# pavlidic/Binary-SpGEMM

Hardware: AMD Instinct MI355X
Metric: output nnz/sec (GNZ/s) (higher is better)
Workload: dtype int32

## Files before the change

binary-spgemm_amd/bspgemm/__init__.py:

```python
import ctypes as C
import os
import subprocess
import weakref

import numpy as np

os.environ.setdefault("OMP_NUM_THREADS", str(min(16, len(os.sched_getaffinity(0)))))
os.environ.setdefault("GPU_MAX_HW_QUEUES", "8")

_PKG = os.path.dirname(os.path.abspath(__file__))
_ROOT = os.path.dirname(_PKG)
LIB_PATH = os.path.join(_ROOT, "libbspgemm.so")

_I32P = np.ctypeslib.ndpointer(dtype=np.int32, flags="C_CONTIGUOUS")
_I64P = np.ctypeslib.ndpointer(dtype=np.int64, flags="C_CONTIGUOUS")

STATUS = {0: "OK", 1: "ERR_INVALID", 2: "ERR_ALLOC", 3: "ERR_HIP", 4: "ERR_NO_DEVICE",
          5: "ERR_OVERFLOW", 6: "ERR_IO", 7: "ERR_FORMAT", 8: "ERR_COMM", 9: "ERR_SIZE"}

EXPORTS = [
    "bspgemm_status_string", "bspgemm_last_error", "bspgemm_create", "bspgemm_destroy",
    "bspgemm_set_stream", "bspgemm_synchronize", "bspgemm_matrix_upload", "bspgemm_matrix_wrap_device",
    "bspgemm_matrix_free", "bspgemm_matrix_rows", "bspgemm_matrix_cols", "bspgemm_matrix_nnz",
    "bspgemm_multiply", "bspgemm_multiply_masked", "bspgemm_result_rows", "bspgemm_result_nnz",
    "bspgemm_result_row_ptr_device", "bspgemm_result_col_idx_device", "bspgemm_result_download",
    "bspgemm_result_free", "bspgemm_row_work_prefix", "bspgemm_partition_rows", "bspgemm_last_stats",
    "SpGEMM_hip", "SpGEMM_hip_bigslice", "SpGEMM_hip_mat", "SpGEMM_hip_masked", "bspgemm_dropin_set_device",
    "bspgemm_comm_unique_id", "bspgemm_comm_create", "bspgemm_comm_destroy", "bspgemm_comm_stitch_row_ptr", "bspgemm_lengths_to_row_ptr",
    "bspgemm_readCOO", "bspgemm_write_mtx", "bspgemm_write_result_mtx", "bspgemm_csr_equal",
    "bspgemm_csr_equal64", "bspgemm_gen_uniform", "bspgemm_gen_rmat", "bspgemm_gen_powerlaw",
    "bspgemm_matrix_from_result", "bspgemm_closure",
    "bspgemm_readCOO_ex", "bspgemm_comm_create_host", "bspgemm_comm_rank", "bspgemm_comm_size",
    "bspgemm_comm_gather_col_idx", "SpGEMM_hip_multi", "bspgemm_device_count", "bspgemm_stats_at",
    "bspgemm_set_flow", "bspgemm_set_class_timing", "bspgemm_build_info", "bspgemm_matrix_invalidate", "bspgemm_comm_agree", "bspgemm_comm_inject_failure",
    "bspgemm_set_option", "bspgemm_get_option", "bspgemm_matrix_uses_blocked_table", "bspgemm_matrix_uses_padded_rows",
]


class BspgemmError(RuntimeError):
    def __init__(self, status, where=""):
        self.status = status
        msg = lib().bspgemm_last_error().decode(errors="replace") if _lib is not None else ""
        super().__init__("%s: %s %s" % (where, STATUS.get(status, status), msg))


MAX_BINS = 20
FLOWS = {"auto": 0, "upper-bound": 1, "exact": 2}
OPTIONS = {"class_streams": 1, "blocked_extents": 2, "check": 3, "small_path": 4, "padded_rows": 5}


class Stats(C.Structure):
    _fields_ = [("rows", C.c_int64), ("nnz_a", C.c_int64), ("products", C.c_int64), ("nnz_c", C.c_int64),
                ("bytes_alg", C.c_int64), ("bytes_read_alg", C.c_int64), ("rows_per_bin", C.c_int64 * MAX_BINS),
                ("ms_total", C.c_float), ("ms_symbolic", C.c_float), ("ms_prepass", C.c_float),
                ("ms_count", C.c_float), ("ms_numeric", C.c_float), ("ms_stitch", C.c_float),
                ("ms_bin", C.c_float * MAX_BINS), ("ms_bin_count", C.c_float * MAX_BINS),
                ("t_bin", C.c_float * MAX_BINS), ("t_bin_count", C.c_float * MAX_BINS), ("bins", C.c_int),
                ("bin_cap", C.c_int * MAX_BINS), ("flow", C.c_int), ("prepass_kernel", C.c_int),
                ("class_streams", C.c_int), ("small_path", C.c_int), ("checked", C.c_int), ("padded_rows", C.c_int)]
# ... 60 lines not shown
    L.bspgemm_set_stream.argtypes = [VP, VP]
    L.bspgemm_synchronize.argtypes = [VP]
    L.bspgemm_set_flow.argtypes = [VP, C.c_int]
    L.bspgemm_set_class_timing.argtypes = [VP, C.c_int]
    L.bspgemm_build_info.restype = C.c_char_p
    L.bspgemm_matrix_invalidate.argtypes = [VP]
    L.bspgemm_set_option.argtypes = [VP, C.c_int, C.c_int]
    L.bspgemm_get_option.argtypes = [VP, C.c_int]
    L.bspgemm_matrix_uses_blocked_table.argtypes = [VP]
    L.bspgemm_matrix_uses_padded_rows.argtypes = [VP]
    L.bspgemm_matrix_upload.argtypes = [VP, C.c_int, C.c_int, VP, VP, PVP]
    L.bspgemm_matrix_wrap_device.argtypes = [VP, C.c_int, C.c_int, C.c_int64, VP, VP, PVP]
    L.bspgemm_matrix_free.argtypes = [VP]
    L.bspgemm_matrix_free.restype = None
    L.bspgemm_matrix_rows.argtypes = [VP]
    L.bspgemm_matrix_cols.argtypes = [VP]
    L.bspgemm_matrix_nnz.argtypes = [VP]
    L.bspgemm_matrix_nnz.restype = C.c_int64
    L.bspgemm_multiply.argtypes = [VP, VP, VP, C.c_int, C.c_int, PVP]
    L.bspgemm_multiply_masked.argtypes = [VP, VP, VP, VP, C.c_int, C.c_int, PVP]
    L.bspgemm_result_rows.argtypes = [VP]
    L.bspgemm_result_nnz.argtypes = [VP]
    L.bspgemm_result_nnz.restype = C.c_int64
    L.bspgemm_result_row_ptr_device.argtypes = [VP]
    L.bspgemm_result_row_ptr_device.restype = VP
    L.bspgemm_result_col_idx_device.argtypes = [VP]
    L.bspgemm_result_col_idx_device.restype = VP
    L.bspgemm_result_download.argtypes = [VP, VP, VP, VP]
    L.bspgemm_result_free.argtypes = [VP]
    L.bspgemm_result_free.restype = None
    L.bspgemm_matrix_from_result.argtypes = [VP, VP, C.c_int, PVP]
    L.bspgemm_closure.argtypes = [VP, VP, C.c_int, PVP, C.POINTER(C.c_int)]
    L.bspgemm_row_work_prefix.argtypes = [VP, VP, VP, _I64P]
    L.bspgemm_partition_rows.argtypes = [VP, VP, VP, C.c_int, _I32P]
    L.bspgemm_last_stats.argtypes = [VP, C.POINTER(Stats)]
    L.bspgemm_stats_at.argtypes = [VP, C.c_int, C.POINTER(Stats)]
    IPP = C.POINTER(C.POINTER(C.c_int))
    L.SpGEMM_hip.argtypes = [_I32P, VP, C.c_int, _I32P, _I32P, C.c_int, IPP, _I32P, C.c_int]
    L.SpGEMM_hip_bigslice.argtypes = [_I32P, _I32P, C.c_int, _I32P, _I32P, C.c_int, IPP, _I32P,
                                      C.POINTER(C.c_int), C.c_int, C.c_int]
    L.SpGEMM_hip_mat.argtypes = [_I32P, _I32P, C.c_int, _I32P, _I32P, C.c_int, _I32P, _I32P]
    L.SpGEMM_hip_masked.argtypes = [_I32P, _I32P, C.c_int, _I32P, _I32P, C.c_int, _I32P, _I32P, IPP, _I32P,
                                    C.POINTER(C.c_int)]
    L.bspgemm_dropin_set_device.argtypes = [C.c_int]
    L.bspgemm_comm_unique_id.argtypes = [C.c_char_p]
    L.bspgemm_comm_create.argtypes = [VP, C.c_char_p, C.c_int, C.c_int, PVP]
    L.bspgemm_comm_destroy.argtypes = [VP]
    L.bspgemm_comm_destroy.restype = None
    L.bspgemm_comm_stitch_row_ptr.argtypes = [VP, VP, _I32P, PVP, VP]
    L.bspgemm_lengths_to_row_ptr.argtypes = [VP, VP, C.c_int, C.c_int, _I32P, VP, VP]
    U32PP = C.POINTER(C.POINTER(C.c_uint32))
    L.bspgemm_readCOO.argtypes = [C.c_char_p, U32PP, U32PP, C.POINTER(C.c_uint32), C.POINTER(C.c_uint32),
                                  C.POINTER(C.c_uint32)]
    L.bspgemm_readCOO_ex.argtypes = [C.c_char_p, C.c_uint, U32PP, U32PP, C.POINTER(C.c_uint32), C.POINTER(C.c_uint32),
                                     C.POINTER(C.c_uint32)]
    L.bspgemm_comm_create_host.argtypes = [VP, C.POINTER(HostTransport), C.c_int, C.c_int, PVP]
    L.bspgemm_comm_rank.argtypes = [VP]
    L.bspgemm_comm_size.argtypes = [VP]
    L.bspgemm_comm_gather_col_idx.argtypes = [VP, VP, _I64P, C.c_int, VP]
    L.SpGEMM_hip_multi.argtypes = [VP, _I32P, _I32P, C.c_int, _I32P, _I32P, C.c_int, IPP, _I32P, C.c_int]
    L.bspgemm_write_mtx.argtypes = [C.c_char_p, C.c_int, C.c_int, _I32P, _I32P]
    L.bspgemm_write_result_mtx.argtypes = [C.c_char_p, C.c_int, C.c_int, _I64P, _I32P]
    L.bspgemm_csr_equal.argtypes = [_I32P, _I32P, _I32P, _I32P, C.c_int]
    L.bspgemm_csr_equal64.argtypes = [_I32P, _I64P, _I32P, _I64P, C.c_int]
    L.bspgemm_gen_uniform.argtypes = [C.c_int, C.c_int, C.c_uint64, IPP, IPP]
    L.bspgemm_gen_rmat.argtypes = [C.c_int, C.c_int, C.c_double, C.c_double, C.c_double, C.c_uint64, IPP, IPP]
# ... 142 lines not shown

    def multiply_masked(self, A, B, F, row_begin=0, row_end=None):
        row_end = A.rows if row_end is None else row_end
        r = C.c_void_p()
        _chk(lib().bspgemm_multiply_masked(self._h, A._h, B._h, F._h, row_begin, row_end, C.byref(r)),
             "bspgemm_multiply_masked")
        return Result(self, r)

    def matrix_from_result(self, result, cols):
        m = C.c_void_p()
        _chk(lib().bspgemm_matrix_from_result(self._h, result._h, cols, C.byref(m)), "matrix_from_result")
        return Matrix(self, m, keep=None)

    def closure(self, A, max_iter=64):
        r, it = C.c_void_p(), C.c_int()
        _chk(lib().bspgemm_closure(self._h, A._h, max_iter, C.byref(r), C.byref(it)), "bspgemm_closure")
        return Result(self, r), it.value

    def lengths_to_row_ptr(self, d_lengths, world, width, bounds, d_row_ptr, hip_stream=None):
        b = np.ascontiguousarray(bounds, dtype=np.int32)
        _chk(lib().bspgemm_lengths_to_row_ptr(self._h, C.c_void_p(int(d_lengths)), int(world), int(width), b,
                                              C.c_void_p(int(d_row_ptr)), C.c_void_p(hip_stream or 0)), "lengths_to_row_ptr")

    def stats(self, age=0):
        s = Stats()
        _chk(lib().bspgemm_stats_at(self._h, age, C.byref(s)), "stats_at")
        return s.as_dict()

    def row_work_prefix(self, A, B):
        out = np.zeros(A.rows + 1, dtype=np.int64)
        _chk(lib().bspgemm_row_work_prefix(self._h, A._h, B._h, out), "row_work_prefix")
        return out

    def partition_rows(self, A, B, parts):
        out = np.zeros(parts + 1, dtype=np.int32)
        _chk(lib().bspgemm_partition_rows(self._h, A._h, B._h, parts, out), "partition_rows")
        return out


class Matrix:
    def __init__(self, ctx, handle, keep):
        self.ctx, self._h, self._keep = ctx, handle, keep
        ctx._children.add(self)
        self.rows = lib().bspgemm_matrix_rows(handle)
        self.cols = lib().bspgemm_matrix_cols(handle)
        self.nnz = lib().bspgemm_matrix_nnz(handle)

    def invalidate(self):
        _chk(lib().bspgemm_matrix_invalidate(self._h), "matrix_invalidate")

    @property
    def uses_blocked_table(self):
        return lib().bspgemm_matrix_uses_blocked_table(self._h)

    @property
    def uses_padded_rows(self):
        return lib().bspgemm_matrix_uses_padded_rows(self._h)

    def free(self):
        if self._h:
            lib().bspgemm_matrix_free(self._h)
            self._h = C.c_void_p()

    def __del__(self):
        try:
            self.free()
# ... 79 lines not shown
```

binary-spgemm_amd/csrc/dense_rows.hip:

```cpp
#include "kernels.hpp"
#include "wave.hpp"
#include <stdlib.h>
#include <type_traits>

namespace bsp {

constexpr int kDenseThreadsBig = 1024;
constexpr int kDenseThreadsMid = 512;
constexpr int kMidMinWaves = 8;
constexpr int kBigMinWaves = 4;
constexpr int kDenseMaxWords = 16384;
constexpr int kMidMaxWords = 4096;
constexpr int kDenseWordBits = 12;
constexpr int kDenseQuadsPerThreadBig = 16;
constexpr int kDenseQuadsPerThreadMid = 8;
constexpr int kDenseInFlightBig = 8;
constexpr int kDenseInFlightMid = 4;

struct __attribute__((packed, aligned(4))) Int4U { int x, y, z, w; };
struct __attribute__((packed, aligned(4))) Int2U { int x, y; };

struct GatherState {
    long long QB = 0;
    bool plan_kept = false;
// ... 6 lines not shown
    static constexpr int kTileQ = kThreads * kQPT;
    static constexpr int kTileWords = kTileQ / 32;
    static_assert(kTileWords % 64 == 0 && kTileWords <= kThreads, "one wave scans the tile's words, blocked");
    int wcnt[kWaves];
    long long wsum[kWaves];
    int2 sd[kThreads];
    u32 tb[kTileWords];
    u32 tw[2][kTileWords];
    int tpre[2][kTileWords];
};

template <int kThreads, int kQPT>
__device__ __forceinline__ void gather_init(GatherLds<kThreads, kQPT> &L)
{
    if ((int)threadIdx.x < GatherLds<kThreads, kQPT>::kTileWords) L.tb[threadIdx.x] = 0u;
}

template <int kThreads, int kQPT, int kInFlight, typename Ins>
__device__ __forceinline__ void gather_sweep(GatherLds<kThreads, kQPT> &L, GatherState &g, const int2 *__restrict__ ab,
                                             const int *__restrict__ Bcol, int nnzB, int a0, int a1, bool first_sweep, Ins ins)
{
    using LT = GatherLds<kThreads, kQPT>;
    constexpr int kWaves = LT::kWaves, kTileQ = LT::kTileQ, kTileWords = LT::kTileWords;
    static_assert(kQPT % kInFlight == 0 && kInFlight % 4 == 0, "whole steps; the last step in quarters");
    const int tid = threadIdx.x, lane = tid & 63, wave = tid >> 6;
    int2 e_next = make_int2(0, 0);
    if (!g.plan_kept && a0 + tid < a1) e_next = ab[a0 + tid];
    for (int ja = a0; ja < a1; ja += kThreads) {
        int2 e = make_int2(0, 0);
        int nq = 0, cidx = 0;
        long long qexcl = 0;
        if (!g.plan_kept) {
            e = e_next;
            e_next = make_int2(0, 0);
            if (ja + kThreads + tid < a1) e_next = ab[ja + kThreads + tid];
            nq = (int)(((u32)e.y + 3u) >> 2);
            const int inc = wave_incl_scan(nq);
            const u64 nonempty = __ballot(nq > 0);
            if (lane == 63) L.wsum[wave] = (long long)inc;
            if (lane == 0) L.wcnt[wave] = __popcll(nonempty);
            __syncthreads();
            qexcl = (long long)(inc - nq);
            g.QB = 0;
            cidx = __popcll(nonempty & mask_lt(lane));
            for (int k = 0; k < kWaves; k++) {
                const long long t = L.wsum[k];
                const int c = L.wcnt[k];
                if (k < wave) { qexcl += t; cidx += c; }
                g.QB += t;
            }
            if (nq > 0) L.sd[cidx] = make_int2((int)((u32)e.x - 4u * (u32)qexcl), e.x + e.y);
            if (g.QB == 0) __syncthreads();
        }
        int carry = -1;
        for (long long T0 = 0; T0 < g.QB; T0 += kTileQ) {
            if (!g.plan_kept) {
                g.buf ^= 1;
                if (nq > 0 && qexcl >= T0 && qexcl < T0 + kTileQ) {
                    const int rel = (int)(qexcl - T0);
                    atomicOr(&L.tb[rel >> 5], 1u << (rel & 31));
                }
                __syncthreads();
                if (wave == 0) {
                    constexpr int WPL = kTileWords / 64;
                    u32 x[WPL];
                    int c[WPL], run = 0;
// ... 677 lines not shown
```

binary-spgemm_amd/csrc/kernels.hpp:

```cpp
#pragma once
#include <hip/hip_runtime.h>
#include <stdint.h>
#include <stdlib.h>

namespace bsp {

constexpr int kWaveBins = 16;
constexpr int kNumBins = kWaveBins + 4;
constexpr int kRankBin = kWaveBins + 1;
constexpr int kMidBin = kWaveBins + 2;
constexpr int kDenseBin = kWaveBins + 3;
constexpr int kRankCap = 6144;
int rank_cap_for_cols(long long cols);
constexpr int kMaxBins = 20;
constexpr int kWaveChunks[kWaveBins + 1] = {0, 1, 2, 3, 4, 5, 6, 7, 8, 10, 12, 14, 16, 20, 24, 28, 32};
constexpr int kMaxWaveCap = 64 * kWaveChunks[kWaveBins];
constexpr int kMidCap = 524288;
inline int mid_cap_for_cols(long long cols)
{
    const long long passes = (cols + (1ll << 18) - 1) >> 18;
    if (passes <= 1) return kMidCap;
    const long long c = kMidCap / passes;
    return c < kMaxWaveCap ? kMaxWaveCap : (int)c;
}
constexpr int kRowsPerWave = 16;

constexpr int kWaveTopWords = 256;

inline int levels_for_cols(int64_t cols)
{
    for (int L = 1; L < 5; L++)
        if (cols <= ((int64_t)kWaveTopWords << (5 * L))) return L;
    return 5;
}

constexpr int kWaveTopWordsWide = 512;
inline int wave_levels_for_cols(int64_t cols)
{
    const int L = levels_for_cols(cols);
    if (L == 4 && cols <= ((int64_t)kWaveTopWordsWide << 15)) return 3;
    return L;
}

struct RowRec {
    int row;
    int a0;
    int alen;
    int f;
};

void launch_row_work(const int *Arow, const int *Acol, const int *Brow, const int *Bblk8, const int *Bpad, const int2 *Bext,
                     int row_begin, int row_end, long long *F, int2 *ab, hipStream_t s);
void launch_blk8(const int *row_ptr, const int *start_ptr, int n, int *blk, unsigned long long *clamped_nnz, hipStream_t s);
void launch_pad_lengths(const int *row_ptr, int n, int *plen, hipStream_t s);
void launch_pad_copy(const int *row_ptr, const int *col_idx, const int *pad_ptr, int n, int *col_pad, int2 *ext, hipStream_t s);

void launch_deg8(const int *row_ptr, int n, unsigned char *deg8, hipStream_t s);
void launch_row_products(const int *Arow, const int *Acol, const int *Brow, const unsigned char *Bdeg8,
                         int row_begin, int row_end, long long *F, hipStream_t s);

struct PrepScalars {
    long long totalF;
    long long heavy_total;
    long long products;
    int a_lo, a_hi;
    int bin_count[kNumBins];
};
void launch_scan_and_bin(const long long *F, int n, int row_begin, const int *Arow, long long *prefix,
                         long long *partials, int *bin_tiles, int *bin_count, RowRec *rec,
                         long long *recpre, int *cnt, int heavy_cols, long long *hpartials, int mid_cap, int rank_cap, int bound_cols,
                         hipStream_t s, PrepScalars *scal = nullptr, const long long *true_F = nullptr);

constexpr int kCompactGran = 4096;
inline size_t compact_chunk_rows(long long max_out) { return (size_t)((max_out + kCompactGran - 1) / kCompactGran) + 2; }
void launch_scan_counts(const int *cnt, int n, long long *prefix, long long *partials,
                        const long long *base, hipStream_t s, int *chunk_row = nullptr);

constexpr unsigned kErrCapacity = 1u;
constexpr unsigned kErrStaleTable = 2u;
void launch_wave_rows(int bin, int levels, const int2 *ab, const int *Bcol, int cols,
                      const RowRec *rec, const long long *recpre, const long long *row_ptr, int nrows,
                      int row_begin, int *tmp, int *cnt, unsigned *err, hipStream_t s, bool count_only = false);
// ... 54 lines not shown
```

binary-spgemm_amd/csrc/multiply.hip:

```cpp
#include "internal.hpp"

using namespace bsp;

static bspgemm_status check_operands(bspgemm_context *ctx, const bspgemm_matrix *A, const bspgemm_matrix *B,
                                     int row_begin, int row_end)
{
    if (!ctx || !A || !B) return FAIL(BSPGEMM_ERR_INVALID, "NULL operand");
    if (A->ctx != ctx || B->ctx != ctx) return FAIL(BSPGEMM_ERR_INVALID, "operand belongs to another context");
    if (row_begin < 0 || row_end < row_begin || row_end > A->rows) return FAIL(BSPGEMM_ERR_INVALID, "row range");
    if (B->rows < A->cols) return FAIL(BSPGEMM_ERR_INVALID, "B has fewer rows than A has columns");
    return BSPGEMM_OK;
}


static void class_order(const int *bin_count, long long total_products, int *order, int *lane)
{
    int light[kWaveBins];
    for (int k = 0; k < kWaveBins; k++) light[k] = k + 1;
    const long long heavy_lower_bound = ((long long)bin_count[kRankBin] + bin_count[kMidBin] + bin_count[kDenseBin]) * kMaxWaveCap;
    if (heavy_lower_bound * 8 < total_products) {
        long long key[kNumBins] = {};
        for (int b = 1; b <= kWaveBins; b++) key[b] = (long long)bin_count[b] * kWaveChunks[b];
        for (int a = 1; a < kWaveBins; a++)
            for (int c = a; c > 0 && key[light[c]] > key[light[c - 1]]; c--) {
// ... 521 lines not shown
        C = next;
        if (C->nnz == prev_nnz) break;
        prev_nnz = C->nnz;
        if (it + 1 == max_iter) break;
        bspgemm_matrix *nm = nullptr;
        st = bspgemm_matrix_from_result(ctx, C, n, &nm);
        if (st) break;
        bspgemm_matrix_free(cur);
        cur = nm;
    }
    bspgemm_matrix_free(cur);
    if (st) { bspgemm_result_free(C); return st; }
    *T = C;
    return BSPGEMM_OK;
}

extern "C" bspgemm_status bspgemm_row_work_prefix(bspgemm_context *ctx, const bspgemm_matrix *A,
                                                  const bspgemm_matrix *B, int64_t *prefix_host)
{
    if (!prefix_host) return FAIL(BSPGEMM_ERR_INVALID, "prefix_host is NULL");
    if (bspgemm_status st = check_operands(ctx, A, B, 0, A ? A->rows : 0)) return st;
    if (bspgemm_status st = use_device(ctx)) return st;
    const int R = A->rows;
    if (bspgemm_status st = ensure_rows(ctx, (size_t)R + 1)) return st;
    if (bspgemm_status st = ensure_deg8(B)) return st;
    launch_row_products(A->d_row_ptr, A->d_col_idx, B->d_row_ptr, B->d_deg8, 0, R, ctx->F, ctx->stream);
    launch_scan_and_bin(ctx->F, R, 0, A->d_row_ptr, ctx->Fprefix, ctx->partials, ctx->bin_tiles, ctx->bin_count,
                        ctx->rec, ctx->recpre, ctx->cnt, 0, nullptr, mid_cap_for_cols(B->cols), rank_cap_for_cols(B->cols), 0, ctx->stream);
    HIPCHK(hipMemcpyAsync(prefix_host, ctx->Fprefix, ((size_t)R + 1) * sizeof(long long), hipMemcpyDeviceToHost, ctx->stream));
    HIPCHK(hipStreamSynchronize(ctx->stream));
    return BSPGEMM_OK;
}

extern "C" bspgemm_status bspgemm_partition_rows(bspgemm_context *ctx, const bspgemm_matrix *A,
                                                 const bspgemm_matrix *B, int parts, int *bounds)
{
    if (!bounds || parts <= 0 || !A) return FAIL(BSPGEMM_ERR_INVALID, "partition_rows");
    const int R = A->rows;
    int64_t *prefix = static_cast<int64_t *>(malloc(((size_t)R + 1) * sizeof(int64_t)));
    if (!prefix) return FAIL(BSPGEMM_ERR_ALLOC, "prefix");
    bspgemm_status st = bspgemm_row_work_prefix(ctx, A, B, prefix);
    if (st == BSPGEMM_OK) {
        const long long per_row = 32;
        const long long total = prefix[R] + per_row * R;
        bounds[0] = 0;
        int r = 0;
        for (int p = 1; p < parts; p++) {
            const long long target = total / parts * p;
            while (r < R && prefix[r] + per_row * r < target) r++;
            bounds[p] = r;
        }
        bounds[parts] = R;
    }
    free(prefix);
    return st;
}
```

binary-spgemm_amd/csrc/prepass.hip:

```cpp
#include "kernels.hpp"
#include "wave.hpp"

namespace bsp {

struct __attribute__((packed, aligned(4))) Int2U { int x, y; };

constexpr int kLongRow = 256;
constexpr int kRowWorkUnroll = 4;
template <typename Sweep>
__device__ __forceinline__ long long rows_of_a_wave(int a0, int a1, int sub, Sweep &&sweep)
{
    const int lane = threadIdx.x & 63;
    long long long_sum = 0;
#pragma unroll
    for (int q = 0; q < 8; q++) {
        const int qa0 = __builtin_amdgcn_readlane(a0, q * 8), qa1 = __builtin_amdgcn_readlane(a1, q * 8);
        if (qa1 - qa0 > kLongRow) {
            long long t = sweep((long long)qa0 + lane, (long long)qa1, 64);
#pragma unroll
            for (int d = 1; d < 64; d <<= 1) t += __shfl_xor(t, d, 64);
            if (lane == q * 8) long_sum = t;
        }
    }
    const bool is_long = a1 - a0 > kLongRow;
    long long sum = is_long ? 0ll : sweep((long long)a0 + sub, (long long)a1, 8);
    sum += __shfl_xor(sum, 1, 64);
    sum += __shfl_xor(sum, 2, 64);
    sum += __shfl_xor(sum, 4, 64);
    return is_long ? long_sum : sum;
}

template <bool PAD>
__global__ __launch_bounds__(256) void k_row_work(const int *__restrict__ Arow,
                                                  const int *__restrict__ Acol,
                                                  const int *__restrict__ Brow,
                                                  const int2 *__restrict__ Bext,
                                                  int row_begin, int nrows,
                                                  long long *__restrict__ F,
                                                  int2 *__restrict__ ab)
{
    const long long gid = (long long)blockIdx.x * blockDim.x + threadIdx.x;
    const int r = (int)(gid >> 3);
    const int sub = (int)(gid & 7);
    int a0 = 0, a1 = 0;
    if (r < nrows) { a0 = Arow[row_begin + r]; a1 = Arow[row_begin + r + 1]; }
    constexpr int U = kRowWorkUnroll;
    auto sweep = [&](long long first, long long end, int stride) {
        long long sum = 0;
        for (long long jj = first; jj < end; jj += (long long)stride * U) {
            int j[U];
#pragma unroll
            for (int u = 0; u < U; u++) j[u] = (jj + stride * u < end) ? Acol[jj + stride * u] : -1;
            Int2U pr[U];
#pragma unroll
            for (int u = 0; u < U; u++) {
                pr[u].x = pr[u].y = 0;
                if (j[u] >= 0) {
                    if (PAD) { const int2 e = Bext[j[u]]; pr[u].x = e.x; pr[u].y = e.x + e.y; }
                    else pr[u] = *reinterpret_cast<const Int2U *>(Brow + j[u]);
                }
            }
#pragma unroll
            for (int u = 0; u < U; u++)
                if (j[u] >= 0) {
                    const int len = pr[u].y - pr[u].x;
                    ab[jj + stride * u] = make_int2(pr[u].x, len);
                    sum += (long long)len;
                }
        }
        return sum;
    };
    const long long sum = rows_of_a_wave(a0, a1, sub, sweep);
    if (r < nrows && sub == 0) F[r] = sum;
}

struct __attribute__((packed, aligned(4))) Blk8 { int base; unsigned lo, hi; };

__global__ __launch_bounds__(256) void k_blk8(const int *__restrict__ row_ptr, const int *__restrict__ start_ptr, int n,
                                              int *__restrict__ blk, unsigned long long *__restrict__ clamped_nnz)
{
    const int b = blockIdx.x * blockDim.x + threadIdx.x;
    if (b * 8 >= n) return;
    const int r0 = b * 8;
    unsigned lo = 0u, hi = 0u;
    long long clamped = 0;
    int prev = row_ptr[r0];
    const int base = start_ptr[r0];
#pragma unroll
    for (int k = 0; k < 8; k++) {
        int d = 0;
        if (r0 + k < n) {
            const int nx = row_ptr[r0 + k + 1];
            d = nx - prev;
            prev = nx;
        }
        const unsigned byte = (unsigned)(d < 255 ? d : 255);
        if (d >= 255) clamped += d;
        if (k < 4) lo |= byte << (8 * k); else hi |= byte << (8 * (k - 4));
    }
    if (clamped > 0) atomicAdd(clamped_nnz, (unsigned long long)clamped);
    blk[3 * b] = base;
    blk[3 * b + 1] = (int)lo;
    blk[3 * b + 2] = (int)hi;
}
void launch_blk8(const int *row_ptr, const int *start_ptr, int n, int *blk, unsigned long long *clamped_nnz, hipStream_t s)
{
    if (n <= 0) return;
    const int nb = (n + 7) / 8;
    hipLaunchKernelGGL(k_blk8, dim3((nb + 255) / 256), dim3(256), 0, s, row_ptr, start_ptr ? start_ptr : row_ptr, n, blk, clamped_nnz);
}

template <bool PAD>
__global__ __launch_bounds__(256) void k_row_work_blk(const int *__restrict__ Arow,
                                                      const int *__restrict__ Acol,
                                                      const int *__restrict__ Brow,
                                                      const int *__restrict__ Bblk,
                                                      const int *__restrict__ Bpad,
                                                      int row_begin, int nrows,
                                                      long long *__restrict__ F,
                                                      int2 *__restrict__ ab)
{
    const long long gid = (long long)blockIdx.x * blockDim.x + threadIdx.x;
    const int r = (int)(gid >> 3);
    const int sub = (int)(gid & 7);
    int a0 = 0, a1 = 0;
    if (r < nrows) { a0 = Arow[row_begin + r]; a1 = Arow[row_begin + r + 1]; }
    constexpr int U = kRowWorkUnroll;
    auto sweep = [&](long long first, long long end, int stride) {
        long long sum = 0;
        for (long long jj = first; jj < end; jj += (long long)stride * U) {
            int j[U];
#pragma unroll
            for (int u = 0; u < U; u++) j[u] = (jj + stride * u < end) ? Acol[jj + stride * u] : -1;
            Blk8 w[U];
#pragma unroll
            for (int u = 0; u < U; u++) {
                w[u].base = 0; w[u].lo = w[u].hi = 0u;
                if (j[u] >= 0) w[u] = *reinterpret_cast<const Blk8 *>(Bblk + 3 * (j[u] >> 3));
            }
            int start[U], len[U];
            bool sat[U];
#pragma unroll
            for (int u = 0; u < U; u++) {
                const int k = j[u] & 7;
                const u64 d = ((u64)w[u].hi << 32) | (u64)w[u].lo;
                const u64 below = d & ((1ull << (8 * k)) - 1ull);
                const u64 upto = (k == 7) ? d : (d & ((1ull << (8 * k + 8)) - 1ull));
                const u64 v = ~upto;
                sat[u] = j[u] >= 0 && ((v - 0x0101010101010101ull) & ~v & 0x8080808080808080ull) != 0ull;
                if (PAD) {
                    const u64 m0f = 0x0f0f0f0f0f0f0f0full, m01 = 0x0101010101010101ull;
                    const u64 units = ((below >> 4) & m0f) + ((((below & m0f) + m0f) >> 4) & m01);
                    start[u] = w[u].base + 16 * ((int)__builtin_amdgcn_sad_u8((unsigned)units, 0u, 0u)
                                                 + (int)__builtin_amdgcn_sad_u8((unsigned)(units >> 32), 0u, 0u));
                } else {
                    start[u] = w[u].base + (int)__builtin_amdgcn_sad_u8((unsigned)below, 0u, 0u)
                               + (int)__builtin_amdgcn_sad_u8((unsigned)(below >> 32), 0u, 0u);
                }
                len[u] = (int)((d >> (8 * k)) & 255ull);
            }
            Int2U pr[U];
            int ps[U];
#pragma unroll
            for (int u = 0; u < U; u++) {
                pr[u].x = pr[u].y = 0;
                ps[u] = 0;
                if (sat[u]) {
                    pr[u] = *reinterpret_cast<const Int2U *>(Brow + j[u]);
                    if (PAD) ps[u] = Bpad[j[u]];
                }
            }
#pragma unroll
            for (int u = 0; u < U; u++)
                if (j[u] >= 0) {
                    if (sat[u]) { start[u] = PAD ? ps[u] : pr[u].x; len[u] = pr[u].y - pr[u].x; }
                    ab[jj + stride * u] = make_int2(start[u], len[u]);
                    sum += (long long)len[u];
                }
        }
        return sum;
    };
    const long long sum = rows_of_a_wave(a0, a1, sub, sweep);
    if (r < nrows && sub == 0) F[r] = sum;
}

void launch_row_work(const int *Arow, const int *Acol, const int *Brow, const int *Bblk8, const int *Bpad, const int2 *Bext,
                     int row_begin, int row_end, long long *F, int2 *ab, hipStream_t s)
{
    const int nrows = row_end - row_begin;
    if (nrows <= 0) return;
    const long long threads = (long long)nrows * 8;
    const int grid = (int)((threads + 255) / 256);
    if (Bblk8 && Bpad)
        hipLaunchKernelGGL(k_row_work_blk<true>, dim3(grid), dim3(256), 0, s, Arow, Acol, Brow, Bblk8, Bpad, row_begin, nrows, F, ab);
    else if (Bblk8)
        hipLaunchKernelGGL(k_row_work_blk<false>, dim3(grid), dim3(256), 0, s, Arow, Acol, Brow, Bblk8, nullptr, row_begin, nrows, F, ab);
    else if (Bext)
        hipLaunchKernelGGL(k_row_work<true>, dim3(grid), dim3(256), 0, s, Arow, Acol, Brow, Bext, row_begin, nrows, F, ab);
    else
        hipLaunchKernelGGL(k_row_work<false>, dim3(grid), dim3(256), 0, s, Arow, Acol, Brow, nullptr, row_begin, nrows, F, ab);
}

__global__ __launch_bounds__(256) void k_pad_lengths(const int *__restrict__ row_ptr, int n, int *__restrict__ plen)
{
    const int i = blockIdx.x * blockDim.x + threadIdx.x;
    if (i < n) plen[i] = ((row_ptr[i + 1] - row_ptr[i]) + 15) & ~15;
}
void launch_pad_lengths(const int *row_ptr, int n, int *plen, hipStream_t s)
{
// ... 14 lines not shown
}
void launch_pad_copy(const int *row_ptr, const int *col_idx, const int *pad_ptr, int n, int *col_pad, int2 *ext, hipStream_t s)
{
    if (n <= 0) return;
    const long long threads = (long long)n * 16;
    hipLaunchKernelGGL(k_pad_copy, dim3((unsigned)((threads + 255) / 256)), dim3(256), 0, s, row_ptr, col_idx, pad_ptr, n, col_pad, ext);
}

__global__ __launch_bounds__(256) void k_deg8(const int *__restrict__ row_ptr, int n, unsigned char *__restrict__ deg8)
{
    const int i = blockIdx.x * blockDim.x + threadIdx.x;
    if (i < n) {
        const int d = row_ptr[i + 1] - row_ptr[i];
        deg8[i] = (unsigned char)(d < 255 ? d : 255);
    }
}
void launch_deg8(const int *row_ptr, int n, unsigned char *deg8, hipStream_t s)
{
    if (n <= 0) return;
    hipLaunchKernelGGL(k_deg8, dim3((n + 255) / 256), dim3(256), 0, s, row_ptr, n, deg8);
}

__global__ __launch_bounds__(256) void k_row_products(const int *__restrict__ Arow, const int *__restrict__ Acol,
                                                      const int *__restrict__ Brow,
                                                      const unsigned char *__restrict__ Bdeg8,
                                                      int row_begin, int nrows, long long *__restrict__ F)
{
    const long long gid = (long long)blockIdx.x * blockDim.x + threadIdx.x;
    const int r = (int)(gid >> 3);
    const int sub = (int)(gid & 7);
    int a0 = 0, a1 = 0;
    if (r < nrows) { a0 = Arow[row_begin + r]; a1 = Arow[row_begin + r + 1]; }
    constexpr int U = 4;
    auto sweep = [&](long long first, long long end, int stride) {
        long long sum = 0;
        for (long long jj = first; jj < end; jj += (long long)stride * U) {
            int j[U];
#pragma unroll
            for (int u = 0; u < U; u++) j[u] = (jj + stride * u < end) ? Acol[jj + stride * u] : -1;
            int d[U];
#pragma unroll
            for (int u = 0; u < U; u++) d[u] = j[u] >= 0 ? (int)Bdeg8[j[u]] : 0;
#pragma unroll
            for (int u = 0; u < U; u++) {
                if (d[u] == 255) d[u] = Brow[j[u] + 1] - Brow[j[u]];
                sum += (long long)d[u];
            }
        }
        return sum;
    };
    const long long sum = rows_of_a_wave(a0, a1, sub, sweep);
    if (r < nrows && sub == 0) F[r] = sum;
}

__global__ __launch_bounds__(256) void k_check_tables(const int *__restrict__ row_ptr, int n,
                                                      const unsigned char *__restrict__ deg8, const int *__restrict__ blk,
                                                      const int *__restrict__ pad_ptr, unsigned *__restrict__ err)
{
    const int i = blockIdx.x * blockDim.x + threadIdx.x;
    if (i >= n) return;
    const int d = row_ptr[i + 1] - row_ptr[i];
    const unsigned want = (unsigned)(d < 255 ? d : 255);
    bool bad = d < 0;
    if (deg8) bad = bad || deg8[i] != want;
    if (blk) {
        const int b = i >> 3, k = i & 7;
        const unsigned w = (unsigned)blk[3 * b + 1 + (k >> 2)];
        bad = bad || ((w >> (8 * (k & 3))) & 255u) != want || (k == 0 && blk[3 * b] != (pad_ptr ? pad_ptr[i] : row_ptr[i]));
    }
    if (pad_ptr) bad = bad || pad_ptr[i + 1] - pad_ptr[i] != ((d + 15) & ~15);
    if (bad) atomicOr(err, kErrStaleTable);
}
// ... 328 lines not shown
```

binary-spgemm_amd/csrc/wave_masked.hip:

```cpp
#include "kernels.hpp"
#include "wave.hpp"

namespace bsp {

constexpr int kMaskWinChunks = 4;
constexpr long long kMaskWaveMaxProducts = 8192;

template <int LEVELS, int CHUNKS>
struct MaskCfg {
    static constexpr int CAP = 64 * CHUNKS;
    static constexpr int TOPW = 256;
    static constexpr int bytes_per_wave = 4 * TOPW + 2 * TOPW + 8 * kMaskWinChunks + 4 * 64
                                          + 4 * CAP * 3
                                          + (LEVELS >= 3 ? 4 * CAP + 2 * CAP : 32)
                                          + 0;
    static constexpr int w4 = (4 * bytes_per_wave > 64 * 1024) ? 0 : (160 * 1024 / (4 * bytes_per_wave)) * 4;
    static constexpr int w2 = (2 * bytes_per_wave > 64 * 1024) ? 0 : (160 * 1024 / (2 * bytes_per_wave)) * 2;
    static constexpr int WAVES = (w4 >= w2 && w4 > 0) ? 4 : (w2 > 0 ? 2 : 1);
};

template <int LEVELS, int CHUNKS>
__global__ __launch_bounds__((64 * MaskCfg<LEVELS, CHUNKS>::WAVES))
void k_wave_masked(const int2 *__restrict__ ab, const int *__restrict__ Bcol, int topw,
                   const int *__restrict__ Frow, const int *__restrict__ Fcol,
// ... 78 lines not shown
            const unsigned short *Ppre = topPre;
#pragma unroll
            for (int lev = LEVELS - 2; lev >= 0; lev--) {
                u32 *S = (lev == 1) ? SB : SA;
                unsigned short *Spre = preB;
#pragma unroll
                for (int c = 0; c < CHUNKS; c++) {
                    const bool ok = c * 64 + lane < mlen;
                    const u32 cc = (u32)mcol[c];
                    const u32 x = P[rank[c]];
                    const int pre = Ppre[rank[c]];
                    const u32 b = (cc >> (5 * (lev + 1))) & 31;
                    const int r2 = pre + __popc(x & ((1u << b) - 1u));
                    if (ok) {
                        atomicOr(&S[r2], 1u << ((cc >> (5 * lev)) & 31));
                        if (lev == 0) L0w[r2] = cc >> 5;
                    }
                    rank[c] = r2;
                }
                wave_lds_fence();
                if (lev > 0) {
                    scan_blocked<CHUNKS>(S, Spre, lane);
                    wave_lds_fence();
                    P = S;
                    Ppre = Spre;
                }
            }
            L0 = SA;
        }

        for (int ab0 = 0; ab0 < alen; ab0 += 64) {
            int2 e = make_int2(0, 0);
            if (ab0 + lane < alen) e = ab[a0 + ab0 + lane];
            const int bs = e.x, len = e.y;
            const int inc = wave_incl_scan(len);
            const int excl = inc - len;
            const int Fb = wave_bcast(inc, 63);
            for (int w0 = 0; w0 < Fb; w0 += 64 * PCH) {
                const bool part = len > 0 && excl < w0 + 64 * PCH && excl + len > w0;
                const u64 bal = __ballot(part);
                if (part) {
                    const int sidx = __popcll(bal & mask_lt(lane));
                    const int pos = (excl > w0 ? excl : w0) - w0;
                    delta[sidx] = bs - excl;
                    atomicOr(&starts[pos >> 6], 1ull << (pos & 63));
                }
                wave_lds_fence();
                u64 sw = 0ull;
                if (lane < PCH) { sw = starts[lane]; starts[lane] = 0ull; }
                const int sinc = wave_incl_scan(__popcll(sw));
                const int sbefore = sinc - __popcll(sw);
                int gaddr[PCH];
#pragma unroll
                for (int c = 0; c < PCH; c++) {
                    const int p = c * 64 + lane;
                    const u64 M = wave_bcast64(sw, c);
                    const int before = wave_bcast(sbefore, c);
                    const bool ok = w0 + p < Fb;
                    int s = before + __popcll(M & mask_le(lane)) - 1;
                    s = ok ? s : 0;
                    gaddr[c] = ok ? delta[s] + w0 + p : 0;
                }
                int pc[PCH];
#pragma unroll
                for (int c = 0; c < PCH; c++) {
                    const bool ok = w0 + c * 64 + lane < Fb;
                    pc[c] = ok ? Bcol[gaddr[c]] : -1;
// ... 134 lines not shown
```

binary-spgemm_amd/csrc/wave_rows.inc:

```
#include "kernels.hpp"
#include "wave.hpp"

namespace bsp {

constexpr int waves_per_cu(int w, int bytes) { return (w * bytes > 64 * 1024) ? 0 : (160 * 1024 / (w * bytes)) * w; }

constexpr int prev_wave_chunks(int chunks)
{
    int prev = 0;
    for (int b = 1; b <= kWaveBins; b++) {
        if (kWaveChunks[b] == chunks) return prev;
        prev = kWaveChunks[b];
    }
    return 0;
}

template <int LEVELS, int CHUNKS, int TWP>
struct WaveCfg {
    static constexpr int CAP = 64 * CHUNKS;
    static constexpr int SW = (CHUNKS <= 2) ? CHUNKS : ((CHUNKS + 3) & ~3);
    static constexpr int SLOTS = 64 * SW;
    static constexpr int TOPW = 64 * TWP;
    static constexpr int bytes_per_wave = 4 * TOPW + 2 * TOPW + 8 * CHUNKS + 4 * SLOTS
                                          + (LEVELS >= 2 ? 4 * SLOTS : 16)
// ... 22 lines not shown
    return make_int2((int)(u32)v, (int)(u32)((u64)v >> 32));
}

constexpr int kMaxAmbiguous = 12;
constexpr int wr_floor_log2(int x) { int k = 0; while ((2 << k) <= x) k++; return k; }

template <int LEVELS, int CHUNKS, int TWP, bool COUNT>
__global__ __launch_bounds__((64 * WaveCfg<LEVELS, CHUNKS, TWP>::WAVES))
void k_wave_rows(const int2 *__restrict__ ab, const int *__restrict__ Bcol,
                 const RowRec *__restrict__ rec, const long long *__restrict__ recpre,
                 const long long *__restrict__ row_ptr,
                 int nrows, int rpw, int row_begin, int *__restrict__ tmp, int *__restrict__ cnt,
                 unsigned *__restrict__ err)
{
    using Cfg = WaveCfg<LEVELS, CHUNKS, TWP>;
    constexpr int TOPW = Cfg::TOPW, WAVES = Cfg::WAVES, SW = Cfg::SW, SLOTS = Cfg::SLOTS, FULL = Cfg::FULL;
    __shared__ __attribute__((aligned(16))) u32 s_top[WAVES][TOPW];
    __shared__ __attribute__((aligned(16))) unsigned short s_topPre[WAVES][TOPW];
    __shared__ __attribute__((aligned(16))) u64 s_starts[WAVES][CHUNKS];
    __shared__ __attribute__((aligned(16))) u32 s_L0w[WAVES][SLOTS];
    __shared__ __attribute__((aligned(16))) u32 s_SA[WAVES][LEVELS >= 2 ? SLOTS : 4];
    __shared__ __attribute__((aligned(16))) u32 s_SB[WAVES][LEVELS >= 3 ? SLOTS : 4];
    __shared__ __attribute__((aligned(16))) unsigned short s_preB[WAVES][LEVELS >= 3 ? SLOTS : 8];
    __shared__ __attribute__((aligned(16))) unsigned short s_preA[WAVES][LEVELS >= 4 ? SLOTS : 8];

    const int lane = lane_id();
    const int plane = (int)(__brev((unsigned)lane) >> 26);
    const int wave_in_wg = threadIdx.x >> 6;
    const long long wave_global = (long long)blockIdx.x * WAVES + wave_in_wg;
    const long long k0 = wave_global * rpw;
    if (k0 >= nrows) return;
    const int nmine = (nrows - k0 < rpw) ? (int)(nrows - k0) : rpw;

    int r_row = 0, r_a0 = 0, r_alen = 0;
    long long r_pre = 0;
    if (lane < nmine) {
        const RowRec q = rec[k0 + lane];
        r_row = q.row;
        r_a0 = q.a0;
        r_alen = q.alen;
        if (!COUNT) r_pre = row_ptr ? row_ptr[q.row - row_begin] : recpre[k0 + lane];
    }

    u32 *top = s_top[wave_in_wg];
    unsigned short *topPre = s_topPre[wave_in_wg];
    u64 *starts = s_starts[wave_in_wg];
    u32 *L0w = s_L0w[wave_in_wg];
    int *delta = reinterpret_cast<int *>(s_L0w[wave_in_wg]);
    u32 *SA = s_SA[wave_in_wg];
    u32 *SB = s_SB[wave_in_wg];
    unsigned short *preA = s_preA[wave_in_wg];
    unsigned short *preB = s_preB[wave_in_wg];

    constexpr int TW = TOPW / 64;
    clear_blocked<TW>(top, lane);
    if (lane < CHUNKS) starts[lane] = 0ull;
    if (LEVELS >= 2) clear_blocked<SW>(SA, lane);
    if (LEVELS >= 3) clear_blocked<SW>(SB, lane);
    wave_lds_fence();

    int2 ab_next = make_int2(0, 0);
    {
        const int a0 = wave_bcast(r_a0, 0), alen = wave_bcast(r_alen, 0);
        if (lane < alen) ab_next = load_extent(ab + a0 + lane);
    }
    if (!COUNT) store_row<CHUNKS, false>(tmp, 0, L0w, lane);

    int my_cnt = 0;
    for (int kk = 0; kk < nmine; kk++) {
        const int a0 = wave_bcast(r_a0, kk);
        const int alen = wave_bcast(r_alen, kk);
        const u32 pre_lo = (u32)wave_bcast((int)(u32)r_pre, kk);
        const u32 pre_hi = (u32)wave_bcast((int)(u32)((unsigned long long)r_pre >> 32), kk);
        int *out = tmp + (long long)(((u64)pre_hi << 32) | pre_lo);

        int F = 0, nsrc = 0;
        for (int ab0 = 0; ab0 < alen; ab0 += 64) {
            int2 e = ab_next;
            if (ab0 > 0) {
                e = make_int2(0, 0);
                if (ab0 + lane < alen) e = load_extent(ab + a0 + ab0 + lane);
            }
            const int bs = e.x, len = e.y;
            const int inc = wave_incl_scan(len);
            const int excl = F + inc - len;
            const u64 bal = __ballot(len > 0);
            if (len > 0 && (unsigned)excl < (unsigned)Cfg::CAP) {
                const int sidx = nsrc + __popcll(bal & mask_lt(lane));
                delta[sidx] = bs - excl;
                atomicOr(&starts[excl >> 6], 1ull << (excl & 63));
            }
            F += wave_bcast(inc, 63);
            nsrc += __popcll(bal);
        }
        if (F > Cfg::CAP || F < 0) {
            if (lane == 0) atomicOr(err, kErrCapacity);
            F = F < 0 ? 0 : Cfg::CAP;
        }
        wave_lds_fence();
        u64 sw = 0ull;
        if (lane < CHUNKS) { sw = starts[lane]; starts[lane] = 0ull; }
        const int sinc = wave_incl_scan(__popcll(sw));
        const int sbefore = sinc - __popcll(sw);

        int col[CHUNKS];
        int rank[CHUNKS];
        int gaddr[CHUNKS];
#pragma unroll
        for (int c = 0; c < CHUNKS; c++) {
            {
                const int p = c * 64 + plane;
                const u64 M = wave_bcast64(sw, c);
                const int before = wave_bcast(sbefore, c);
                int s = before + __popcll(M & mask_le(plane)) - 1;
                s = (c < FULL || p < F) ? s : 0;
                gaddr[c] = delta[s];
            }
        }
#pragma unroll
        for (int c = 0; c < CHUNKS; c++) {
            {
                const int p = c * 64 + plane;
                const int g = gaddr[c] + ((c < FULL || p < F) ? p : 0);
                col[c] = Bcol[g];
            }
        }
        ab_next = make_int2(0, 0);
        if (kk + 1 < nmine) {
            const int na0 = wave_bcast(r_a0, kk + 1), nalen = wave_bcast(r_alen, kk + 1);
            if (lane < nalen) ab_next = load_extent(ab + na0 + lane);
        }
        wave_lds_fence();

        bool row_counted = false;
        int running = 0;
        if constexpr (COUNT && LEVELS >= 2 && CHUNKS <= 16) {
            constexpr int HB = wr_floor_log2(32 * SLOTS);
            u32 *hb = SA;
            bool amb[CHUNKS];
            u64 am[CHUNKS];
            int namb = 0;
#pragma unroll
            for (int c = 0; c < CHUNKS; c++) {
                const bool ok = c < FULL || c * 64 + plane < F;
                const u32 cc = (u32)col[c];
                const u32 h = (cc ^ (cc >> HB) ^ (2 * HB < 32 ? cc >> ((2 * HB) & 31) : 0u)) & ((1u << HB) - 1u);
                u32 old = 0u;
// ... 207 lines not shown
```

include/bspgemm.h:

```cpp
#ifndef BSPGEMM_H
#define BSPGEMM_H

#include <stddef.h>
#include <stdint.h>

#ifdef __cplusplus
extern "C" {
#endif

typedef enum bspgemm_status {
    BSPGEMM_OK            = 0,
    BSPGEMM_ERR_INVALID   = 1,
    BSPGEMM_ERR_ALLOC     = 2,
    BSPGEMM_ERR_HIP       = 3,
    BSPGEMM_ERR_NO_DEVICE = 4,
    BSPGEMM_ERR_OVERFLOW  = 5,
    BSPGEMM_ERR_IO        = 6,
    BSPGEMM_ERR_FORMAT    = 7,
    BSPGEMM_ERR_COMM      = 8,
    BSPGEMM_ERR_SIZE      = 9
} bspgemm_status;

const char *bspgemm_status_string(bspgemm_status s);
const char *bspgemm_last_error(void);
// ... 36 lines not shown
    BSPGEMM_OPT_CLASS_STREAMS   = 1,
    BSPGEMM_OPT_BLOCKED_EXTENTS = 2,
    BSPGEMM_OPT_CHECK           = 3,
    BSPGEMM_OPT_SMALL_PATH      = 4,
    BSPGEMM_OPT_PADDED_ROWS     = 5
} bspgemm_option;
bspgemm_status bspgemm_set_option(bspgemm_context *ctx, bspgemm_option opt, int value);
int            bspgemm_get_option(const bspgemm_context *ctx, bspgemm_option opt);
int            bspgemm_matrix_uses_blocked_table(const bspgemm_matrix *m);
int            bspgemm_matrix_uses_padded_rows(const bspgemm_matrix *m);

bspgemm_status bspgemm_multiply_masked(bspgemm_context *ctx,
                                       const bspgemm_matrix *A, const bspgemm_matrix *B,
                                       const bspgemm_matrix *F,
                                       int row_begin, int row_end, bspgemm_result **C);

int            bspgemm_result_rows(const bspgemm_result *C);
int64_t        bspgemm_result_nnz(const bspgemm_result *C);
const int64_t *bspgemm_result_row_ptr_device(const bspgemm_result *C);
const int     *bspgemm_result_col_idx_device(const bspgemm_result *C);
bspgemm_status bspgemm_result_download(bspgemm_context *ctx, const bspgemm_result *C,
                                       int64_t *row_ptr, int *col_idx);
void           bspgemm_result_free(bspgemm_result *C);

bspgemm_status bspgemm_matrix_from_result(bspgemm_context *ctx, const bspgemm_result *C, int cols,
                                          bspgemm_matrix **out);

bspgemm_status bspgemm_closure(bspgemm_context *ctx, const bspgemm_matrix *A, int max_iter,
                               bspgemm_result **T, int *iterations);

bspgemm_status bspgemm_row_work_prefix(bspgemm_context *ctx,
                                       const bspgemm_matrix *A, const bspgemm_matrix *B,
                                       int64_t *prefix_host );
bspgemm_status bspgemm_partition_rows(bspgemm_context *ctx,
                                      const bspgemm_matrix *A, const bspgemm_matrix *B,
                                      int parts, int *bounds);

#define BSPGEMM_MAX_BINS 20
typedef struct bspgemm_stats {
    int64_t rows;
    int64_t nnz_a;
    int64_t products;
    int64_t nnz_c;
    int64_t bytes_alg;
    int64_t bytes_read_alg;
    int64_t rows_per_bin[BSPGEMM_MAX_BINS];
    float   ms_total;
    float   ms_symbolic;
    float   ms_prepass;
    float   ms_count;
    float   ms_numeric;
    float   ms_stitch;
    float   ms_bin[BSPGEMM_MAX_BINS];
    float   ms_bin_count[BSPGEMM_MAX_BINS];
    float   t_bin[BSPGEMM_MAX_BINS];
    float   t_bin_count[BSPGEMM_MAX_BINS];
    int     bins;
    int     bin_cap[BSPGEMM_MAX_BINS];
    int     flow;
    int     prepass_kernel;
    int     class_streams;
    int     small_path;
    int     checked;
    int     padded_rows;
} bspgemm_stats;
bspgemm_status bspgemm_last_stats(const bspgemm_context *ctx, bspgemm_stats *out);
// ... 76 lines not shown
```

Measured before the change: 217.7.

## Precompute per-row exclusive offsets in row-work prepass and drop wave scans

```diff
diff --git a/binary-spgemm_amd/bspgemm/__init__.py b/binary-spgemm_amd/bspgemm/__init__.py
--- a/binary-spgemm_amd/bspgemm/__init__.py
+++ b/binary-spgemm_amd/bspgemm/__init__.py
@@ -24,7 +24,7 @@
     "bspgemm_matrix_free", "bspgemm_matrix_rows", "bspgemm_matrix_cols", "bspgemm_matrix_nnz",
     "bspgemm_multiply", "bspgemm_multiply_masked", "bspgemm_result_rows", "bspgemm_result_nnz",
     "bspgemm_result_row_ptr_device", "bspgemm_result_col_idx_device", "bspgemm_result_download",
-    "bspgemm_result_free", "bspgemm_row_work_prefix", "bspgemm_partition_rows", "bspgemm_last_stats",
+    "bspgemm_result_free", "bspgemm_row_work_prefix", "bspgemm_row_extents", "bspgemm_partition_rows", "bspgemm_last_stats",
     "SpGEMM_hip", "SpGEMM_hip_bigslice", "SpGEMM_hip_mat", "SpGEMM_hip_masked", "bspgemm_dropin_set_device",
     "bspgemm_comm_unique_id", "bspgemm_comm_create", "bspgemm_comm_destroy", "bspgemm_comm_stitch_row_ptr", "bspgemm_lengths_to_row_ptr",
     "bspgemm_readCOO", "bspgemm_write_mtx", "bspgemm_write_result_mtx", "bspgemm_csr_equal",
@@ -151,6 +151,7 @@
     L.bspgemm_matrix_from_result.argtypes = [VP, VP, C.c_int, PVP]
     L.bspgemm_closure.argtypes = [VP, VP, C.c_int, PVP, C.POINTER(C.c_int)]
     L.bspgemm_row_work_prefix.argtypes = [VP, VP, VP, _I64P]
+    L.bspgemm_row_extents.argtypes = [VP, VP, VP, _I32P]
     L.bspgemm_partition_rows.argtypes = [VP, VP, VP, C.c_int, _I32P]
     L.bspgemm_last_stats.argtypes = [VP, C.POINTER(Stats)]
     L.bspgemm_stats_at.argtypes = [VP, C.c_int, C.POINTER(Stats)]
@@ -359,6 +360,11 @@
         _chk(lib().bspgemm_row_work_prefix(self._h, A._h, B._h, out), "row_work_prefix")
         return out
 
+    def row_extents(self, A, B):
+        out = np.zeros(2 * A.nnz, dtype=np.int32)
+        _chk(lib().bspgemm_row_extents(self._h, A._h, B._h, out), "row_extents")
+        return out.reshape(-1, 2)
+
     def partition_rows(self, A, B, parts):
         out = np.zeros(parts + 1, dtype=np.int32)
         _chk(lib().bspgemm_partition_rows(self._h, A._h, B._h, parts, out), "partition_rows")
diff --git a/binary-spgemm_amd/csrc/dense_rows.hip b/binary-spgemm_amd/csrc/dense_rows.hip
--- a/binary-spgemm_amd/csrc/dense_rows.hip
+++ b/binary-spgemm_amd/csrc/dense_rows.hip
@@ -62,6 +62,7 @@
         long long qexcl = 0;
         if (!g.plan_kept) {
             e = e_next;
+            e.y = ab_len(e.y);
             e_next = make_int2(0, 0);
             if (ja + kThreads + tid < a1) e_next = ab[ja + kThreads + tid];
             nq = (int)(((u32)e.y + 3u) >> 2);
diff --git a/binary-spgemm_amd/csrc/kernels.hpp b/binary-spgemm_amd/csrc/kernels.hpp
--- a/binary-spgemm_amd/csrc/kernels.hpp
+++ b/binary-spgemm_amd/csrc/kernels.hpp
@@ -48,6 +48,10 @@
     int alen;
     int f;
 };
+
+constexpr int kAbExclLimit = 1 << 15;
+__host__ __device__ __forceinline__ int ab_len(int y) { return y < 0 ? (y & 0x7fffffff) : (y & 0xffff); }
+__host__ __device__ __forceinline__ int ab_excl(int y) { return (int)((unsigned)y >> 16); }
 
 void launch_row_work(const int *Arow, const int *Acol, const int *Brow, const int *Bblk8, const int *Bpad, const int2 *Bext,
                      int row_begin, int row_end, long long *F, int2 *ab, hipStream_t s);
diff --git a/binary-spgemm_amd/csrc/multiply.hip b/binary-spgemm_amd/csrc/multiply.hip
--- a/binary-spgemm_amd/csrc/multiply.hip
+++ b/binary-spgemm_amd/csrc/multiply.hip
@@ -577,6 +577,26 @@
     return BSPGEMM_OK;
 }
 
+extern "C" bspgemm_status bspgemm_row_extents(bspgemm_context *ctx, const bspgemm_matrix *A, const bspgemm_matrix *B,
+                                              int32_t *ab_host)
+{
+    if (!ab_host) return FAIL(BSPGEMM_ERR_INVALID, "ab_host is NULL");
+    if (bspgemm_status st = check_operands(ctx, A, B, 0, A ? A->rows : 0)) return st;
+    if (bspgemm_status st = use_device(ctx)) return st;
+    const int R = A->rows;
+    if (bspgemm_status st = ensure_rows(ctx, (size_t)R + 1)) return st;
+    if (bspgemm_status st = ensure_ab(ctx, (size_t)A->nnz + 1)) return st;
+    if (bspgemm_status st = ensure_pad(B)) return st;
+    if (bspgemm_status st = ensure_blk8(B)) return st;
+    launch_row_work(A->d_row_ptr, A->d_col_idx, B->d_row_ptr, B->blk8_state == 1 ? B->d_blk8 : nullptr,
+                    B->pad_state == 1 ? B->d_row_ptr_pad : nullptr, B->pad_state == 1 ? B->d_ext : nullptr, 0, R,
+                    ctx->F, ctx->ab, ctx->stream);
+    if (A->nnz > 0)
+        HIPCHK(hipMemcpyAsync(ab_host, ctx->ab, (size_t)A->nnz * sizeof(int2), hipMemcpyDeviceToHost, ctx->stream));
+    HIPCHK(hipStreamSynchronize(ctx->stream));
+    return BSPGEMM_OK;
+}
+
 extern "C" bspgemm_status bspgemm_partition_rows(bspgemm_context *ctx, const bspgemm_matrix *A,
                                                  const bspgemm_matrix *B, int parts, int *bounds)
 {
diff --git a/binary-spgemm_amd/csrc/prepass.hip b/binary-spgemm_amd/csrc/prepass.hip
--- a/binary-spgemm_amd/csrc/prepass.hip
+++ b/binary-spgemm_amd/csrc/prepass.hip
@@ -1,3 +1,4 @@
+#include <type_traits>
 #include "kernels.hpp"
 #include "wave.hpp"
 
@@ -16,18 +17,55 @@
     for (int q = 0; q < 8; q++) {
         const int qa0 = __builtin_amdgcn_readlane(a0, q * 8), qa1 = __builtin_amdgcn_readlane(a1, q * 8);
         if (qa1 - qa0 > kLongRow) {
-            long long t = sweep((long long)qa0 + lane, (long long)qa1, 64);
+            long long t = sweep(std::integral_constant<int, 64>(), (long long)qa0, (long long)qa1, lane);
 #pragma unroll
             for (int d = 1; d < 64; d <<= 1) t += __shfl_xor(t, d, 64);
             if (lane == q * 8) long_sum = t;
         }
     }
     const bool is_long = a1 - a0 > kLongRow;
-    long long sum = is_long ? 0ll : sweep((long long)a0 + sub, (long long)a1, 8);
+    long long sum = is_long ? 0ll : sweep(std::integral_constant<int, 8>(), (long long)a0, (long long)a1, sub);
     sum += __shfl_xor(sum, 1, 64);
     sum += __shfl_xor(sum, 2, 64);
     sum += __shfl_xor(sum, 4, 64);
     return is_long ? long_sum : sum;
+}
+
+template <int G>
+__device__ __forceinline__ int group_incl_scan(int x, int idx)
+{
+    if constexpr (G == 64) {
+        return wave_incl_scan(x);
+    } else {
+        static_assert(G == 8, "groups of 8 or 64 lanes");
+        int t = __builtin_amdgcn_update_dpp(0, x, 0x111, 0xF, 0xF, false);
+        x += idx >= 1 ? t : 0;
+        t = __builtin_amdgcn_update_dpp(0, x, 0x112, 0xF, 0xF, false);
+        x += idx >= 2 ? t : 0;
+        t = __builtin_amdgcn_update_dpp(0, x, 0x114, 0xF, 0xF, false);
+        x += idx >= 4 ? t : 0;
+        return x;
+    }
+}
+template <int G>
+__device__ __forceinline__ int group_last(int x)
+{
+    if constexpr (G == 64) return __builtin_amdgcn_readlane(x, 63);
+    else return __shfl(x, G - 1, G);
+}
+
+template <int G, int U>
+__device__ __forceinline__ void ab_encode(const int (&len)[U], int (&y)[U], int &run, int idx)
+{
+#pragma unroll
+    for (int u = 0; u < U; u++) {
+        const int lc = len[u] < 0 ? 0 : (len[u] > 0xffff ? 0xffff : len[u]);
+        const int inc = group_incl_scan<G>(lc, idx);
+        const int excl = run + inc - lc;
+        y[u] = ((unsigned)len[u] < 0x10000u && excl < kAbExclLimit) ? ((excl << 16) | len[u]) : (int)(0x80000000u | (u32)len[u]);
+        const int tot = run + group_last<G>(inc);
+        run = tot < 0x10000 ? tot : 0x10000;
+    }
 }
 
 template <bool PAD>
@@ -45,12 +83,15 @@
     int a0 = 0, a1 = 0;
     if (r < nrows) { a0 = Arow[row_begin + r]; a1 = Arow[row_begin + r + 1]; }
     constexpr int U = kRowWorkUnroll;
-    auto sweep = [&](long long first, long long end, int stride) {
+    auto sweep = [&](auto Gc, long long base, long long end, int idx) {
+        constexpr int G = decltype(Gc)::value;
         long long sum = 0;
-        for (long long jj = first; jj < end; jj += (long long)stride * U) {
+        int run = 0;
+        for (long long jb = base; jb < end; jb += (long long)G * U) {
+            const long long jj = jb + idx;
             int j[U];
 #pragma unroll
-            for (int u = 0; u < U; u++) j[u] = (jj + stride * u < end) ? Acol[jj + stride * u] : -1;
+            for (int u = 0; u < U; u++) j[u] = (jj + G * u < end) ? Acol[jj + G * u] : -1;
             Int2U pr[U];
 #pragma unroll
             for (int u = 0; u < U; u++) {
@@ -60,12 +101,15 @@
                     else pr[u] = *reinterpret_cast<const Int2U *>(Brow + j[u]);
                 }
             }
+            int len[U], y[U];
+#pragma unroll
+            for (int u = 0; u < U; u++) len[u] = pr[u].y - pr[u].x;
+            ab_encode<G, U>(len, y, run, idx);
 #pragma unroll
             for (int u = 0; u < U; u++)
                 if (j[u] >= 0) {
-                    const int len = pr[u].y - pr[u].x;
-                    ab[jj + stride * u] = make_int2(pr[u].x, len);
-                    sum += (long long)len;
+                    ab[jj + G * u] = make_int2(pr[u].x, y[u]);
+                    sum += (long long)len[u];
                 }
         }
         return sum;
@@ -126,12 +170,15 @@
     int a0 = 0, a1 = 0;
     if (r < nrows) { a0 = Arow[row_begin + r]; a1 = Arow[row_begin + r + 1]; }
     constexpr int U = kRowWorkUnroll;
-    auto sweep = [&](long long first, long long end, int stride) {
+    auto sweep = [&](auto Gc, long long base, long long end, int idx) {
+        constexpr int G = decltype(Gc)::value;
         long long sum = 0;
-        for (long long jj = first; jj < end; jj += (long long)stride * U) {
+        int run = 0;
+        for (long long jb = base; jb < end; jb += (long long)G * U) {
+            const long long jj = jb + idx;
             int j[U];
 #pragma unroll
-            for (int u = 0; u < U; u++) j[u] = (jj + stride * u < end) ? Acol[jj + stride * u] : -1;
+            for (int u = 0; u < U; u++) j[u] = (jj + G * u < end) ? Acol[jj + G * u] : -1;
             Blk8 w[U];
 #pragma unroll
             for (int u = 0; u < U; u++) {
@@ -171,10 +218,16 @@
                 }
             }
 #pragma unroll
+            for (int u = 0; u < U; u++) {
+                if (sat[u]) { start[u] = PAD ? ps[u] : pr[u].x; len[u] = pr[u].y - pr[u].x; }
+                if (j[u] < 0) len[u] = 0;
+            }
+            int y[U];
+            ab_encode<G, U>(len, y, run, idx);
+#pragma unroll
             for (int u = 0; u < U; u++)
                 if (j[u] >= 0) {
-                    if (sat[u]) { start[u] = PAD ? ps[u] : pr[u].x; len[u] = pr[u].y - pr[u].x; }
-                    ab[jj + stride * u] = make_int2(start[u], len[u]);
+                    ab[jj + G * u] = make_int2(start[u], y[u]);
                     sum += (long long)len[u];
                 }
         }
@@ -255,12 +308,13 @@
     int a0 = 0, a1 = 0;
     if (r < nrows) { a0 = Arow[row_begin + r]; a1 = Arow[row_begin + r + 1]; }
     constexpr int U = 4;
-    auto sweep = [&](long long first, long long end, int stride) {
+    auto sweep = [&](auto Gc, long long base, long long end, int idx) {
+        constexpr int G = decltype(Gc)::value;
         long long sum = 0;
-        for (long long jj = first; jj < end; jj += (long long)stride * U) {
+        for (long long jj = base + idx; jj < end; jj += (long long)G * U) {
             int j[U];
 #pragma unroll
-            for (int u = 0; u < U; u++) j[u] = (jj + stride * u < end) ? Acol[jj + stride * u] : -1;
+            for (int u = 0; u < U; u++) j[u] = (jj + G * u < end) ? Acol[jj + G * u] : -1;
             int d[U];
 #pragma unroll
             for (int u = 0; u < U; u++) d[u] = j[u] >= 0 ? (int)Bdeg8[j[u]] : 0;
diff --git a/binary-spgemm_amd/csrc/wave_masked.hip b/binary-spgemm_amd/csrc/wave_masked.hip
--- a/binary-spgemm_amd/csrc/wave_masked.hip
+++ b/binary-spgemm_amd/csrc/wave_masked.hip
@@ -134,7 +134,7 @@
         for (int ab0 = 0; ab0 < alen; ab0 += 64) {
             int2 e = make_int2(0, 0);
             if (ab0 + lane < alen) e = ab[a0 + ab0 + lane];
-            const int bs = e.x, len = e.y;
+            const int bs = e.x, len = ab_len(e.y);
             const int inc = wave_incl_scan(len);
             const int excl = inc - len;
             const int Fb = wave_bcast(inc, 63);
diff --git a/binary-spgemm_amd/csrc/wave_rows.inc b/binary-spgemm_amd/csrc/wave_rows.inc
--- a/binary-spgemm_amd/csrc/wave_rows.inc
+++ b/binary-spgemm_amd/csrc/wave_rows.inc
@@ -78,13 +78,14 @@
     if (k0 >= nrows) return;
     const int nmine = (nrows - k0 < rpw) ? (int)(nrows - k0) : rpw;
 
-    int r_row = 0, r_a0 = 0, r_alen = 0;
+    int r_row = 0, r_a0 = 0, r_alen = 0, r_f = 0;
     long long r_pre = 0;
     if (lane < nmine) {
         const RowRec q = rec[k0 + lane];
         r_row = q.row;
         r_a0 = q.a0;
         r_alen = q.alen;
+        r_f = q.f;
         if (!COUNT) r_pre = row_ptr ? row_ptr[q.row - row_begin] : recpre[k0 + lane];
     }
 
@@ -120,23 +121,21 @@
         const u32 pre_hi = (u32)wave_bcast((int)(u32)((unsigned long long)r_pre >> 32), kk);
         int *out = tmp + (long long)(((u64)pre_hi << 32) | pre_lo);
 
-        int F = 0, nsrc = 0;
+        int F = wave_bcast(r_f, kk);
+        int nsrc = 0;
         for (int ab0 = 0; ab0 < alen; ab0 += 64) {
             int2 e = ab_next;
             if (ab0 > 0) {
                 e = make_int2(0, 0);
                 if (ab0 + lane < alen) e = load_extent(ab + a0 + ab0 + lane);
             }
-            const int bs = e.x, len = e.y;
-            const int inc = wave_incl_scan(len);
-            const int excl = F + inc - len;
+            const int bs = e.x, len = e.y & 0xffff, excl = ab_excl(e.y);
             const u64 bal = __ballot(len > 0);
             if (len > 0 && (unsigned)excl < (unsigned)Cfg::CAP) {
                 const int sidx = nsrc + __popcll(bal & mask_lt(lane));
                 delta[sidx] = bs - excl;
                 atomicOr(&starts[excl >> 6], 1ull << (excl & 63));
             }
-            F += wave_bcast(inc, 63);
             nsrc += __popcll(bal);
         }
         if (F > Cfg::CAP || F < 0) {
@@ -146,19 +145,18 @@
         wave_lds_fence();
         u64 sw = 0ull;
         if (lane < CHUNKS) { sw = starts[lane]; starts[lane] = 0ull; }
-        const int sinc = wave_incl_scan(__popcll(sw));
-        const int sbefore = sinc - __popcll(sw);
 
         int col[CHUNKS];
         int rank[CHUNKS];
         int gaddr[CHUNKS];
+        int before = -1;
 #pragma unroll
         for (int c = 0; c < CHUNKS; c++) {
             {
                 const int p = c * 64 + plane;
                 const u64 M = wave_bcast64(sw, c);
-                const int before = wave_bcast(sbefore, c);
-                int s = before + __popcll(M & mask_le(plane)) - 1;
+                int s = before + __popcll(M & mask_le(plane));
+                before += __popcll(M);
                 s = (c < FULL || p < F) ? s : 0;
                 gaddr[c] = delta[s];
             }
diff --git a/include/bspgemm.h b/include/bspgemm.h
--- a/include/bspgemm.h
+++ b/include/bspgemm.h
@@ -92,6 +92,9 @@
 bspgemm_status bspgemm_row_work_prefix(bspgemm_context *ctx,
                                        const bspgemm_matrix *A, const bspgemm_matrix *B,
                                        int64_t *prefix_host );
+bspgemm_status bspgemm_row_extents(bspgemm_context *ctx,
+                                   const bspgemm_matrix *A, const bspgemm_matrix *B,
+                                   int32_t *ab_host );
 bspgemm_status bspgemm_partition_rows(bspgemm_context *ctx,
                                       const bspgemm_matrix *A, const bspgemm_matrix *B,
                                       int parts, int *bounds);
```

Measured after the change: 219.9 (median of 6 runs). Within noise of the previous version (+1.0%).
